# HENDRIX-ZT2/pyaudiorestoration

Measured on AMD Instinct MI355X. Metric: Msamples/sec resampled (192 kHz varispeed), higher is better.
Workload: dtype f32 near taps, far taps (|n| >= 3) as float16 hi + lo x 2^-12 filter banks on v_mfma_f32_16x16x32_f16 with f32 accumulation / f64 positions

## Files before the change

pyaudiorestoration_amd/csrc/sinc2.hip:

```cpp
#define PAR_WANT_BANK2 1
#include "par_common.h"
#include "pos_plan.h"
#include "sinc_taps_gen.h"
#include "sinc_common.h"
#define PAR_COLD_FN __forceinline__
#include "sinc_block.h"
#ifndef PAR_COLD_FN_GIVEN
#error "sinc_block.h was included before PAR_COLD_FN was defined: the cold functions would stay out of line"
#endif
#include <algorithm>
#include <atomic>
#include <limits.h>
#include <type_traits>

constexpr int kMaxTilesPerWave = 23;
#ifndef PAR_S2_EXP
#define PAR_S2_EXP 0
#endif

namespace par {

typedef _Float16 half8v __attribute__((ext_vector_type(8)));
typedef _Float16 half2v __attribute__((ext_vector_type(2)));
typedef float float4v __attribute__((ext_vector_type(4)));
// ... 138 lines not shown
  _Float16 img[2 * NCH][kRingH];
  float4v qa[kPass];
  float4v qm0[MOM ? kPass : kPass / 4];
  float4v qm1[MOM ? kPass : 1];
  __device__ __forceinline__ float& e2d2(int sl) {
    return MOM ? reinterpret_cast<float*>(&qm0[sl])[3] : reinterpret_cast<float*>(&qm0[0])[sl];
  }
  __device__ __forceinline__ const float& e2d2(int sl) const {
    return MOM ? reinterpret_cast<const float*>(&qm0[sl])[3] : reinterpret_cast<const float*>(&qm0[0])[sl];
  }
#ifdef PAR_S3_LDS_PAD
  uint4 pad[PAR_S3_LDS_PAD / 16];
#endif
  uint4 recs[4][16];
};
static_assert(offsetof(S3Lds<1>, img) % 16 == 0 && offsetof(S3Lds<1>, qa) % 16 == 0 && offsetof(S3Lds<1>, recs) % 16 == 0, "16-byte aligned");
static_assert(offsetof(S3Lds<2>, ring) % 16 == 0 && offsetof(S3Lds<2>, img) % 16 == 0 && offsetof(S3Lds<2>, qa) % 16 == 0 &&
              offsetof(S3Lds<2>, recs) % 16 == 0, "16-byte aligned");
static_assert(sizeof(S3Lds<2>) <= 20480, "eight stereo streams per compute unit (160 KB of LDS)");
using S3LdsUnity = S3Lds<1, false>;
static_assert(sizeof(S3LdsUnity) <= 10240 && offsetof(S3LdsUnity, recs) % 16 == 0 && offsetof(S3LdsUnity, qa) % 16 == 0,
              "sixteen fc = 1 streams per compute unit");

struct S3Pass {
  int cw[2];
  float s[2], ep[2];
  int nok[2];
  int j, ws;
};

constexpr int kCtabUnity = 10;
struct S3Frags {
  half8v xh[3], xl[3];
};
template <class LDS>
__device__ __forceinline__ S3Frags bank_load(const LDS& L, const int offs, const int l, const int ch = 0) {
  const int bb = l & 15, g = l >> 4;
  const int i0 = offs + 8 * bb + 8 * g;
  S3Frags X;
#pragma unroll
  for (int ks = 0; ks < 3; ++ks) {
    const int ix = (i0 + 32 * ks) & (kRingH - 1);
    X.xh[ks] = *reinterpret_cast<const half8v*>(&L.img[2 * ch][ix]);
    X.xl[ks] = *reinterpret_cast<const half8v*>(&L.img[2 * ch + 1][ix]);
  }
  return X;
}
template <bool MOMENTS, bool SIX = true, class LDS>
__device__ __forceinline__ void bank_math(LDS& L, const half8v (&fr)[kBank2Frags], const half8v (&fmr)[kBank3Frags],
                                          const S3Frags& X, const int l) {
  const int bb = l & 15, g = l >> 4;
  const half8v (&xh)[3] = X.xh, (&xl)[3] = X.xl;
  auto frag = [&](int f) { return f < kCtabUnity ? fr[f] : fmr[f - kCtabUnity]; };
  const float4v z = {0.0f, 0.0f, 0.0f, 0.0f};
  float4v e0 = z, lo = z, e1 = z, e2 = z;
#pragma unroll
  for (int ks = 0; ks < 3; ++ks) {
    const half8v f0 = frag(ks);
    e0 = __builtin_amdgcn_mfma_f32_16x16x32_f16(f0, xh[ks], e0, 0, 0, 0);
    lo = __builtin_amdgcn_mfma_f32_16x16x32_f16(frag(5 + ks), xh[ks], lo, 0, 0, 0);
    lo = __builtin_amdgcn_mfma_f32_16x16x32_f16(f0, xl[ks], lo, 0, 0, 0);
    if (ks < 2) {
      const half8v f1 = frag(3 + ks);
      e1 = __builtin_amdgcn_mfma_f32_16x16x32_f16(f1, xh[ks], e1, 0, 0, 0);
      e2 = __builtin_amdgcn_mfma_f32_16x16x32_f16(frag(8 + ks), xh[ks], e2, 0, 0, 0);
    }
  }
  float lo_inv = kBank2LoInv;
  asm volatile("" : "+v"(lo_inv));
  const float4v v0 = e0 + lo * lo_inv, v1 = e1;
  float4v a01 = z, l01 = z, a23 = z, a45 = z, a6 = z;
  if (MOMENTS) {
#pragma unroll
    for (int ks = 0; ks < 3; ++ks) {
      const half8v f01 = frag(kCtabUnity + ks);
      a01 = __builtin_amdgcn_mfma_f32_16x16x32_f16(f01, xh[ks], a01, 0, 0, 0);
      l01 = __builtin_amdgcn_mfma_f32_16x16x32_f16(frag(kCtabUnity + 3 + ks), xh[ks], l01, 0, 0, 0);
      l01 = __builtin_amdgcn_mfma_f32_16x16x32_f16(f01, xl[ks], l01, 0, 0, 0);
      a23 = __builtin_amdgcn_mfma_f32_16x16x32_f16(frag(kCtabUnity + 6 + ks), xh[ks], a23, 0, 0, 0);
      a45 = __builtin_amdgcn_mfma_f32_16x16x32_f16(frag(kCtabUnity + 9 + ks), xh[ks], a45, 0, 0, 0);
      if constexpr (SIX) a6 = __builtin_amdgcn_mfma_f32_16x16x32_f16(frag(kCtabUnity + 12 + ks), xh[ks], a6, 0, 0, 0);
    }
  }
  const float4v m01 = a01 + l01 * lo_inv;
#pragma unroll
  for (int p = 0; p < 2; ++p) {
    const int sl = (8 * bb + 2 * g + p) ^ (bb & 7);
    const float4v row = {v0[2 * p], v0[2 * p + 1], v1[2 * p], v1[2 * p + 1]};
    L.qa[sl] = row;
    const float e2d2 = __uint_as_float(pack_h2(e2[2 * p] * 0.015625f, e2[2 * p + 1] * 0.015625f));
    if constexpr (MOMENTS) {
      const float4v r0 = {m01[2 * p], m01[2 * p + 1], a23[2 * p], e2d2};
      L.qm0[sl] = r0;
      const float4v r1 = {a23[2 * p + 1], a45[2 * p], a45[2 * p + 1], a6[2 * p]};
      L.qm1[sl] = r1;
    } else {
      L.e2d2(sl) = e2d2;
    }
  }
}
template <bool MOMENTS, bool SIX = true, class LDS>
__device__ __forceinline__ void bank_image3m(LDS& L, const half8v (&fr)[kBank2Frags], const half8v (&fmr)[kBank3Frags],
                                             const int offs, const int l, const int ch = 0) {
  bank_math<MOMENTS, SIX>(L, fr, fmr, bank_load(L, offs, l, ch), l);
}

struct S3Gather {
  float4v row, M0, Mh;
  float xm2, xm1, x0, xp1, xp2;
};
template <int MODE, int NCH = 1, class LDS>
__device__ __forceinline__ S3Gather s3_out_load(const LDS& L, const int ci, const int wsK, const int ch = 0) {
  const int sl = ci ^ ((ci >> 3) & 7);
  const int rc = (wsK + ci) & (kRingF - 1);
  const float* xp = &L.ring[NCH * rc + ch];
  S3Gather G;
  G.xm2 = xp[-2 * NCH], G.xm1 = xp[-NCH], G.x0 = xp[0], G.xp1 = xp[NCH], G.xp2 = xp[2 * NCH];
  G.row = L.qa[sl];
  G.M0 = float4v{0.0f, 0.0f, 0.0f, 0.0f};
  G.Mh = G.M0;
  if constexpr (MODE != 1) {
    G.M0 = L.qm0[sl];
    G.Mh = L.qm1[sl];
  } else {
    G.M0[3] = L.e2d2(sl);
  }
  return G;
}
template <int MODE>
__device__ __forceinline__ float s3_out_math(const S3Gather& Gr, const float sr, const float epr) {
  using T32 = TapTab<32>;
  constexpr float kUs = kBank2ScaleInv * kImgScaleInv;
  constexpr float kMs = kImgScaleInv;
  const float xm2 = Gr.xm2, xm1 = Gr.xm1, x0 = Gr.x0, xp1 = Gr.xp1, xp2 = Gr.xp2;
  const float q = sr * sr, q64 = 64.0f * q;
  const float R1 = fast_rcp(fmaf(q, T32::B[1], T32::A[1])), R2 = fast_rcp(fmaf(q, T32::B[2], T32::A[2]));
  {
// ... 142 lines not shown
                                         jw, nrem, piece);
    else if (nrem > 0)
      fused_wave<NCH, 32, 2 * NCH, false>(a.len_out, a.sig, a.sig + 1, NCH, a.len_in, 32, a.tab, a.tmd, a.out, a.out + 1, NCH, a.fa, piece, l,
                                          jw, nrem, piece);
    return;
    }
  }
  const int64_t stream_id = (int64_t)bx - a.n_edge;
  const int my_tiles = stream_id < a.n_big ? a.tiles : a.tiles_tail;
  const int64_t Ta = stream_id < a.n_big ? stream_id * a.tiles : a.n_big * a.tiles + (stream_id - a.n_big) * a.tiles_tail;
  if (Ta >= a.n_full) return;
  const int64_t Tb = Ta + my_tiles < a.n_full ? Ta + my_tiles : a.n_full;
  const int64_t Ja = Ta * kSincTileOutputs, Jb = Tb * kSincTileOutputs;
  long long A0;
  int hd_dA, hd_fl;
  {
    const int64_t Ti = Ta + l < a.n_tiles ? Ta + l : a.n_tiles - 1;
    const TileHdr h = a.hdr[l <= my_tiles ? Ti : Ta];
    A0 = (long long)(((unsigned long long)(unsigned)__builtin_amdgcn_readfirstlane((int)((unsigned long long)h.anchor >> 32)) << 32) |
                     (unsigned)__builtin_amdgcn_readfirstlane((int)(unsigned)(unsigned long long)h.anchor));
    const long long d = h.anchor - A0;
    hd_fl = h.flags | ((d > -0x40000000ll && d < 0x40000000ll) ? 0 : 1);
    if (a.n_edge > 0 && (Ta + l == 0 || Ta + l >= a.n_full - 2)) hd_fl |= 1 | kTileEdge;
    hd_dA = (int)d;
    if constexpr (KIND == 1 || KIND == 2) {
      const bool any_slow = __ballot(l < my_tiles && Ta + l < Tb && (h.flags & kTileMaySlow) != 0) != 0ull;
      if (any_slow != (KIND == 2)) return;
    }
  }
  half8v fr[kBank2Frags];
  {
    const uint4* src = reinterpret_cast<const uint4*>(kBank2Frags32) + l;
#pragma unroll
    for (int f = 0; f < kBank2Frags; ++f) fr[f] = __builtin_bit_cast(half8v, src[f * kWave]);
  }
  half8v fmr[kBank3Frags];
  if constexpr (kMom) {
    const uint4* src = reinterpret_cast<const uint4*>(kBank3Frags32) + l;
#pragma unroll
    for (int f = 0; f < kBank3Frags; ++f) fmr[f] = __builtin_bit_cast(half8v, src[f * kWave]);
  }
  {
    uint4* z = reinterpret_cast<uint4*>(&L.img[0][0]);
    const uint4 zero = {0u, 0u, 0u, 0u};
#pragma unroll
    for (int i = 0; i < (int)(sizeof(L.img) / 16 / kWave); ++i) z[i * kWave + l] = zero;
  }
  const float tolf = (float)((fabs((double)A0) + 2.0e7) * 1.2e-16 + 2.0e-10) + 2.0e-7f;
  const int nJ = (int)(Jb - Ja);
  float* const outW = a.out + (kPick ? a.out_stride : (int64_t)NCH) * Ja;
  const uint4* const recW = reinterpret_cast<const uint4*>(a.rec) + (Ja >> kRecShift);
  const uint4* const rec2W = reinterpret_cast<const uint4*>(a.rec2) + (Ja >> kRecShift);
  const int blk_max = (int)(((a.len_out + kRec - 1) >> kRecShift) - (Ja >> kRecShift)) - 1;

  int j0 = 0;
  constexpr int kDmaBadMax = 1 << 22;
  int wbase = 0, conv_next = 0, conv_lo = 0, dma_next = 0, dma_bad = 0, mode = 0, pk = 0;
  int regime = 1;
  int rbA = 0, rbB = 0, rbC = 0;

  const uint4* const rec_lane = (l < 8 ? recW : rec2W) + (l & 7);
  using LdsT = S3Lds<NCH, KIND != 1>;
  const unsigned lds_base = lds_addr(&L);
  const unsigned lds_recs = lds_base + (unsigned)offsetof(LdsT, recs), lds_ring = lds_base + (unsigned)offsetof(LdsT, ring);
  constexpr unsigned kRecBufBytes = 16 * sizeof(uint4);
  constexpr unsigned kChunkBytes = kPass * NCH * sizeof(float);
  auto fetch_records_at = [&](unsigned rbytes, int blk0) {
    if (l < 16) dma_dwordx4(rec_lane + (blk0 < 0 ? 0 : blk0), lds_recs + rbytes);
  };
  auto fetch_records = [&](int buf, int blk0) { fetch_records_at(kRecBufBytes * (unsigned)buf, blk0); };
  unsigned long long ring_src = (unsigned long long)(uintptr_t)a.sig;
  auto ring_restart = [&]() {
    const long long o = A0 + wbase;
    ring_src = (unsigned long long)(uintptr_t)a.sig + (unsigned long long)((long long)(NCH * sizeof(float)) * o);
// ... 108 lines not shown
                "the largest stream (48 tiles of stereo frames) stays below 2^32 bytes");
  auto out_bytes = [&](auto elem, int j) -> size_t { return (size_t)(((unsigned)j + (unsigned)l) * (unsigned)sizeof(elem)); };
  auto store_pass = [&](const S3Pass& Q, const float (&res)[2]) {
#pragma unroll
    for (int r = 0; r < 2; ++r)
      if (l < Q.nok[r] && !(PAR_S2_EXP & 4)) {
        if constexpr (kPick) outW[(int64_t)((unsigned)Q.j + 64u * r + (unsigned)l) * a.out_stride] = res[r];
        else *reinterpret_cast<float*>(reinterpret_cast<char*>(outW) + out_bytes(float{}, Q.j) + kWave * sizeof(float) * r) = res[r];
      }
  };
  auto store_pass2 = [&](const S3Pass& Q, const float (&res0)[2], const float (&res1)[2]) {
#pragma unroll
    for (int r = 0; r < 2; ++r)
      if (l < Q.nok[r] && !(PAR_S2_EXP & 4))
        *reinterpret_cast<float2*>(reinterpret_cast<char*>(outW) + out_bytes(float2{}, Q.j) + kWave * sizeof(float2) * r) = make_float2(res0[r], res1[r]);
  };
  auto convert_chunk = [&](int w0) -> unsigned long long {
    if constexpr (kPick) {
      return s3_convert_ch(L, w0, l, 0, true);
    } else if constexpr (NCH == 2) {
      const unsigned long long t0 = s3_convert_ch(L, w0, l, 0, true);
      const unsigned long long t1 = s3_convert_ch(L, w0, l, 1, false);
      return t0 | t1;
    } else {
      return s3_convert(L, w0, l);
    }
  };

#if PAR_S2_EXP & 128
#define S3_COUNT(k) do { if (l == 0) atomicAdd(a.redo_count + (k), 1); } while (0)
#else
#define S3_COUNT(k) do { } while (0)
#endif
  auto start_run = [&]() -> bool {
    for (;;) {
      if (j0 >= nJ) return false;
      S3_COUNT(1);
      __builtin_amdgcn_s_waitcnt(0x0F70);
      wave_lds_fence();
      const int buf = pk & 3;
      fetch_records(buf, j0 >> kRecShift);
      __builtin_amdgcn_s_waitcnt(0x0F70);
      wave_lds_fence();
      const Placed Q = place(j0, buf, j0 >> kRecShift);
      const int tend = Q.tend;
      int nv[2] = {clamp64(nJ - j0), clamp64(nJ - j0 - 64)};
      const unsigned long long b0 = __ballot(Q.R[0].bad() || !(Q.R[0].ep <= kEpMaxMom)) & prefix(nv[0]),
                               b1 = __ballot(Q.R[1].bad() || !(Q.R[1].ep <= kEpMaxMom)) & prefix(nv[1]);
      const int nt0 = clamp64(Q.nt[0]), nt1 = clamp64(Q.nt[1]);
      const unsigned long long bad_here = (b0 & prefix(nt0)) | (b1 & prefix(nt1));
      const bool bad_next = ((b0 & ~prefix(nt0)) | (b1 & ~prefix(nt1)) | (unsigned long long)((Q.fl1 & 1) && tend < nJ)) != 0ull;
      if (bad_next) {
        nv[0] = nv[0] < nt0 ? nv[0] : nt0;
        nv[1] = nv[1] < nt1 ? nv[1] : nt1;
      }
      bool skip = (Q.fl0 & 1) || bad_here != 0ull;
      const unsigned long long gen = (__ballot(1.0f + Q.R[0].ep != 1.0f) & prefix(nv[0])) | (__ballot(1.0f + Q.R[1].ep != 1.0f) & prefix(nv[1]));
      const int ws = __builtin_amdgcn_readfirstlane(Q.R[0].c) & ~7;
      S3Pass N;
#pragma unroll
      for (int r = 0; r < 2; ++r) {
        N.cw[r] = Q.R[r].c - ws;
        N.s[r] = Q.R[r].s;
        N.ep[r] = Q.R[r].ep;
        const unsigned long long in = __ballot(N.cw[r] < kPass);
        N.nok[r] = __popcll(in & prefix(nv[r]));
      }
      N.j = j0;
      N.ws = ws;
// ... 27 lines not shown
        while (dma_next < conv_end + 2) chunk_dma(dma_next++);
        const int jn = j0 + N.nok[0] + N.nok[1];
        rbA = jn >> kRecShift;
        rbB = (jn + 120) >> kRecShift;
        fetch_records((pk + 1) & 3, rbA);
        fetch_records((pk + 2) & 3, rbB);
        __builtin_amdgcn_s_waitcnt(0x0F70);
        wave_lds_fence();
        if (!skip) {
#pragma unroll 1
          while (conv_next < conv_end) {
            if (conv_next >= dma_bad) {
              skip = true;
              break;
            }
            const bool ok = convert_chunk(kPass * conv_next) == 0ull;
            if (!ok) {
              skip = true;
              break;
            }
            ++conv_next;
          }
        }
        if (!skip && conv_next + 1 >= dma_bad) skip = true;
      }
      if (skip) {
        if (!(Q.fl0 & kTileEdge)) push_tile(Ta + (j0 >> 10));
        j0 = tend;
        mode = 0;
        continue;
      }
      wave_lds_fence();
      const int offs = ws - wbase - 31;
      if (kMom && regime == 3) bank_image3m<kMom, true>(L, fr, fmr, offs, l);
      else if (kMom && regime == 2) bank_image3m<kMom, false>(L, fr, fmr, offs, l);
      else bank_image3m<false>(L, fr, fmr, offs, l);
      wave_lds_fence();
      j0 += N.nok[0] + N.nok[1];
      ++pk;
      rbC = (j0 + 240) >> kRecShift;
      const bool full = N.nok[1] >= 1 && N.nok[0] + N.nok[1] >= 120;
      if (full) {
        P = N;
        return true;
      }
      float res[2];
      if (kMom && regime == 3) out_pass(std::integral_constant<int, kMom ? 3 : 1>{}, N, res);
      else if (kMom && regime == 2) out_pass(std::integral_constant<int, kMom ? 2 : 1>{}, N, res);
      else out_pass(std::integral_constant<int, 1>{}, N, res);
      if constexpr (kTwo) {
        float res1[2];
        wave_lds_fence();
        if (regime == 3) bank_image3m<true, true>(L, fr, fmr, offs, l, 1);
        else if (regime == 2) bank_image3m<true, false>(L, fr, fmr, offs, l, 1);
        else bank_image3m<false>(L, fr, fmr, offs, l, 1);
        wave_lds_fence();
        if (regime == 3) out_pass(std::integral_constant<int, 3>{}, N, res1, 1);
        else if (regime == 2) out_pass(std::integral_constant<int, 2>{}, N, res1, 1);
        else out_pass(std::integral_constant<int, 1>{}, N, res1, 1);
        store_pass2(N, res, res1);
      } else {
        store_pass(N, res);
      }
    }
  };

#if PAR_S2_EXP & 64
  unsigned long long s3t_[4] = {0, 0, 0, 0}, s3last_ = __builtin_readcyclecounter();
  const unsigned long long s3start_ = s3last_;
#endif
  auto hot = [&](auto mode_tag) {
    constexpr int MODE = decltype(mode_tag)::value;
    j0 = __builtin_amdgcn_readfirstlane(j0);
    wbase = __builtin_amdgcn_readfirstlane(wbase);
    rbA = __builtin_amdgcn_readfirstlane(rbA);
    rbB = __builtin_amdgcn_readfirstlane(rbB);
    rbC = __builtin_amdgcn_readfirstlane(rbC);
    tc_tend = __builtin_amdgcn_readfirstlane(tc_tend);
    tc_flm = __builtin_amdgcn_readfirstlane(tc_flm);
    const int cn0 = __builtin_amdgcn_readfirstlane(conv_next), pk0 = __builtin_amdgcn_readfirstlane(pk);
    const int dn0 = __builtin_amdgcn_readfirstlane(dma_next), dbad = __builtin_amdgcn_readfirstlane(dma_bad);
    int w0 = kPass * cn0;
    unsigned rbytes = kRecBufBytes * (unsigned)(pk0 & 3);
    unsigned dslot = kChunkBytes * (unsigned)(dn0 & 7);
    unsigned long long dsrc = ring_src + (unsigned long long)((long long)kChunkBytes * dn0);
    dsrc = ((unsigned long long)(unsigned)__builtin_amdgcn_readfirstlane((int)(dsrc >> 32)) << 32) |
           (unsigned)__builtin_amdgcn_readfirstlane((int)(unsigned)dsrc);
    const int nJm = nJ - kPass;
    const int cn_lim = kPass * (dbad - 2);
    const int dn_lim = kPass * (dbad - (dn0 - cn0));
    unsigned long long cok = 0ull;
    int m = 0, adv = 0;
    for (;;) {
#if PAR_S2_EXP & 64
      const unsigned long long tA_ = __builtin_readcyclecounter();
#endif
      if constexpr (NCH == 2) asm volatile("s_waitcnt vmcnt(7)" ::: "memory");
      else asm volatile("s_waitcnt vmcnt(5)" ::: "memory");
#if PAR_S2_EXP & 64
      const unsigned long long tB_ = __builtin_readcyclecounter();
      s3t_[0] += tB_ - tA_;
      s3t_[1] += tA_ - s3last_;
      s3last_ = tB_;
      s3t_[2] += 1;
#endif
// ... 18 lines not shown
        N.nok[r] = __popcll(__ballot(N.cw[r] < kPass));
      }
      N.j = j0;
      N.ws = ws;
      wsK = ws - wbase;
      const int d = w0 - wsK;
      auto smin = [](int x, int y) {
        int r = min(x, y);
        asm volatile("" : "+s"(r));
        return r;
      };
      adv = N.nok[0] + N.nok[1];
      m = smin(tc_flm, nJm - j0);
      m = smin(m, adv - 120 - 16 * n_none);
      m = smin(m, smin(d - 161, 473 - d));
      m = smin(m, cn_lim - w0);
      m = smin(m, smin(jb, 1 - jb));
      if constexpr (MODE != 1) m = smin(m, n_some - 1);
      };
      float res[2];
      if constexpr (kEarly) {
        const PlaceRecs RR = place_load(j0, rbytes, jb);
        const float2 cxx = s3_convert_load(L, w0, l);
        S3Gather G[2];
        const int wsP = P.ws - wbase;
#pragma unroll
        for (int r = 0; r < 2; ++r) {
          int ci = P.cw[r];
          ci = ci < 0 ? 0 : (ci > kPass - 1 ? kPass - 1 : ci);
          G[r] = s3_out_load<MODE, NCH>(L, ci, wsP);
        }
        __builtin_amdgcn_sched_barrier(0);
        place_next(std::true_type{}, RR);
        const S3Frags X = bank_load(L, wsK - 31, l);
        __builtin_amdgcn_sched_barrier(0);
        if constexpr (MODE == 2) {
          res[0] = s3_out_math<MODE>(G[0], P.s[0], P.ep[0]);
          asm volatile("" : "+v"(res[0]));
          asm volatile("" ::"v"(G[0].Mh[3]));
          __builtin_amdgcn_sched_barrier(0);
          res[1] = s3_out_math<MODE>(G[1], P.s[1], P.ep[1]);
          bank_math<true, false>(L, fr, fmr, X, l);
          asm volatile("" : "+v"(res[1]));
          asm volatile("" ::"v"(G[1].Mh[3]));
#pragma unroll
          for (int i = 0; i < 28; ++i) {
            __builtin_amdgcn_sched_group_barrier(0x008, 1, 0);
            __builtin_amdgcn_sched_group_barrier(0x002, 2, 0);
          }
        } else {
#pragma unroll
          for (int r = 0; r < 2; ++r) res[r] = s3_out_math<MODE>(G[r], P.s[r], P.ep[r]);
          asm volatile("" : "+v"(res[0]), "+v"(res[1]));
          __builtin_amdgcn_sched_barrier(0);
          bank_math<MODE != 1, MODE == 3>(L, fr, fmr, X, l);
        }
        cok = s3_convert_math(L, w0, l, cxx);
        fetch_records_at(rbytes ^ (2 * kRecBufBytes), rbC);
        chunk_dma_at(w0 < dn_lim, dsrc, dslot);
        store_pass(P, res);
      } else {
      if constexpr (!kTwo) place_next(std::false_type{}, PlaceRecs{});
      out_pass(mode_tag, P, res);
      if constexpr (kTwo) {
        float res1[2];
        asm volatile("" : "+v"(res[0]), "+v"(res[1]));
        bank_image3m<MODE != 1, MODE == 3>(L, fr, fmr, P.ws - wbase - 31, l, 1);
        out_pass(mode_tag, P, res1, 1);
        asm volatile("" : "+v"(res1[0]), "+v"(res1[1]));
        place_next(std::false_type{}, PlaceRecs{});
        const int offs = wsK - 31;
        bank_image3m<MODE != 1, MODE == 3>(L, fr, fmr, offs, l, 0);
        const unsigned long long c0 = s3_convert_ch(L, w0, l, 0, true);
        const unsigned long long c1 = s3_convert_ch(L, w0 - kPass, l, 1, false);
        cok = c0 | c1;
        fetch_records_at(rbytes ^ (2 * kRecBufBytes), rbC);
        chunk_dma_at(w0 < dn_lim, dsrc, dslot);
        store_pass2(P, res, res1);
      } else {
        const int offs = wsK - 31;
#if PAR_S3_PIN_MONO
        asm volatile("" : "+v"(res[0]), "+v"(res[1]));
#endif
        bank_image3m<MODE != 1, MODE == 3>(L, fr, fmr, offs, l);
        cok = convert_chunk(w0);
        fetch_records_at(rbytes ^ (2 * kRecBufBytes), rbC);
        chunk_dma_at(w0 < dn_lim, dsrc, dslot);
        store_pass(P, res);
      }
      }
      wave_lds_fence();
      w0 += kPass;
      dsrc += kChunkBytes;
      dslot = (dslot + kChunkBytes) & (8 * kChunkBytes - 1);
      S3_COUNT(2);
      if (min(m, -(int)__popcll(cok)) < 0) break;
      P = N;
      j0 += adv;
      rbytes = (rbytes + kRecBufBytes) & (3 * kRecBufBytes);
      rbA = rbB;
      rbB = rbC;
      rbC = (j0 + 240) >> kRecShift;
    }
    conv_next = w0 >> 7;
    dma_next = dn0 + (conv_next - cn0);
    pk = pk0 + (conv_next - cn0) - 1;
    if (cok != 0ull) mode = 0;
    if constexpr (kTwo)
      if (mode != 0 && s3_convert_ch(L, w0 - kPass, l, 1, false) != 0ull) mode = 0;
  };

  while (start_run()) {
    if (kMom && regime == 3) hot(std::integral_constant<int, kMom ? 3 : 1>{});
    else if (kMom && regime == 2) hot(std::integral_constant<int, kMom ? 2 : 1>{});
    else hot(std::integral_constant<int, 1>{});
  }
  __builtin_amdgcn_s_waitcnt(0x0F70);
#if PAR_S2_EXP & 64
  if (l == 0) {
    unsigned long long* o = g_s2_phase + (size_t)stream_id * 16;
    o[0] = s3t_[0];
    o[1] = s3t_[1];
    o[2] = s3t_[2];
    o[3] = __builtin_readcyclecounter() - s3start_;
    o[6] = s3t_[2];
  }
#endif
}

template <int NCH, int KIND>
__global__ __launch_bounds__(kWave, KIND == 1 ? 3 : 2) void k_sinc_pipe(const S2Args a) {
  __shared__ S3Lds<NCH, KIND != 1> L;
  sinc_pipe_body<NCH, KIND>(a, (int)blockIdx.x, L);
}

constexpr int kBatchFiles = kFusedBatchMax;
struct S2Batch {
  int n;
  int first[kBatchFiles + 1];
  S2Args f[kBatchFiles];
};
static_assert(sizeof(S2Batch) <= 3584, "kernel arguments fit the 4 KB segment");
template <int NCH, int KIND>
__global__ __launch_bounds__(kWave, KIND == 1 ? 3 : 2) void k_sinc_pipe_n(const S2Batch b) {
  __shared__ S3Lds<NCH, KIND != 1> L;
  const int bx = (int)blockIdx.x;
  int fi = 0;
// ... 107 lines not shown
```

pyaudiorestoration_amd/csrc/sinc_taps_gen.h:

```cpp
#pragma once

namespace par {

template <int NT> struct TapTab;

template <> struct TapTab<32> {
  static constexpr int p1_from = 9, p0_from = 25;
  static constexpr int mode[33] = {0, 0, 0, 0, 0, 1, 1, 1, 1, 2, 2, 2, 2, 2, 2, 2, 2, 2, 2, 2, 2, 2, 2, 2, 2, 3, 3, 3, 3, 3, 3, 3, 3};
  static constexpr float A[33] = {0.0f, 3.149174690246582f, 12.688271522521973f, 28.89647102355957f, 52.254295349121094f, -0.011980682611465454f, 0.008096873760223389f, -0.005758844781666994f, 0.0042452262714505196f, -0.0032113760244101286f, 0.0024757650680840015f, -0.001935371314175427f, 0.0015282001113519073f, -0.0012151190312579274f, 0.0009704310796223581f, -0.000776688102632761f, 0.0006216989131644368f, -0.0004967301501892507f, 0.0003953868872486055f, -0.0003128938842564821f, 0.0002456224465277046f, -0.00019077055912930518f, 0.00014614294923376292f, -0.00010999643563991413f, 8.092952339211479e-05f, -5.7813980674836785e-05f, 3.9685513911535963e-05f, -2.5783318051253445e-05f, 1.5455205357284285e-05f, -8.15003295429051e-06f, 3.398380613361951e-06f, -7.97579900790879e-07f, 0.0f};
  static constexpr float B[33] = {-3.1415927410125732f, -3.149174690246582f, -3.172067880630493f, -3.210718870162964f, -3.2658934593200684f, -0.00047922731027938426f, 0.00022491315030492842f, -0.00011752743739634752f, 6.633166049141437e-05f, -3.976941297878511e-05f, 2.481971932866145e-05f, -1.6027928722905926e-05f, 1.0630960787239019e-05f, -7.2007073868007865e-06f, 4.957503279001685e-06f, -3.4557874641905073e-06f, 2.4308856154675595e-06f, -1.7202777371494449e-06f, 1.221272327711631e-06f, -8.673427487337904e-07f, 6.144401254459808e-07f, -4.328316833834833e-07f, 3.0210429713406484e-07f, -2.0803109634925931e-07f, 1.40563656714221e-07f, 0.0f, 0.0f, 0.0f, 0.0f, 0.0f, 0.0f, 0.0f, 0.0f};
  static constexpr float C[33] = {0.0f, 0.0f, 0.0f, 0.0f, 0.0f, -1.916909241117537e-05f, 6.247587862162618e-06f, -2.398519200141891e-06f, 1.0364321951783495e-06f, 0.0f, 0.0f, 0.0f, 0.0f, 0.0f, 0.0f, 0.0f, 0.0f, 0.0f, 0.0f, 0.0f, 0.0f, 0.0f, 0.0f, 0.0f, 0.0f, 0.0f, 0.0f, 0.0f, 0.0f, 0.0f, 0.0f, 0.0f, 0.0f};
};

template <> struct TapTab<50> {
  static constexpr int p1_from = 9, p0_from = 37;
  static constexpr int mode[51] = {0, 0, 0, 0, 0, 1, 1, 1, 1, 2, 2, 2, 2, 2, 2, 2, 2, 2, 2, 2, 2, 2, 2, 2, 2, 2, 2, 2, 2, 2, 2, 2, 2, 2, 2, 2, 2, 3, 3, 3, 3, 3, 3, 3, 3, 3, 3, 3, 3, 3, 3};
  static constexpr float A[51] = {0.0f, 3.144695281982422f, 12.616111755371094f, 28.526979446411133f, 51.06767654418945f, -0.01242081169039011f, 0.008531484752893448f, -0.006186992395669222f, 0.004665991757065058f, -0.0036238711327314377f, 0.0028791376389563084f, -0.0023288081865757704f, 0.0019109291024506092f, -0.0015864137094467878f, 0.0013296125689521432f, -0.0011231281096115708f, 0.000954821880441159f, -0.0008160152356140316f, 0.0007003697683103383f, -0.0006031683878973126f, 0.0005208412767387927f, -0.00045064662117511034f, 0.0003904495679307729f, -0.0003385677409823984f, 0.00029366035596467555f, -0.0002546478935983032f, 0.00022065313532948494f, -0.0001909568381961435f, 0.0001649646437726915f, -0.0001421815832145512f, 0.00012219262134749442f, -0.00010464734805282205f, 8.924811118049547e-05f, -7.574055780423805e-05f, 6.39061036054045e-05f, -5.355593020794913e-05f, 4.452605207916349e-05f, -3.667675264296122e-05f, 2.987515108543448e-05f, -2.4015091184992343e-05f, 1.8998915038537234e-05f, -1.473993052059086e-05f, 1.1160883332195226e-05f, -8.192681889340747e-06f, 5.773316843260545e-06f, -3.846952040476026e-06f, 2.3631571366422577e-06f, -1.2762477581418352e-06f, 5.447275839287613e-07f, -1.3080894234462903e-07f, 0.0f};
  static constexpr float B[51] = {-3.1415927410125732f, -3.144695281982422f, -3.1540279388427734f, -3.1696643829345703f, -3.191729784011841f, -0.0004968324792571366f, 0.0002369856956647709f, -0.00012626514944713563f, 7.290612120414153e-05f, -4.4877713662572205e-05f, 2.8863558327429928e-05f, -1.9286206224933267e-05f, 1.3293425581650808e-05f, -9.400972885487135e-06f, 6.792402928113006e-06f, -4.9972336455539335e-06f, 3.7334193621063605e-06f, -2.826027184710256e-06f, 2.163304543500999e-06f, -1.6719844779800042e-06f, 1.3029175534029491e-06f, -1.0224540574199636e-06f, 8.071309025581286e-07f, -6.403172392310807e-07f, 5.10048380419903e-07f, -4.075996855590347e-07f, 3.265307384481275e-07f, -2.6203341008113057e-07f, 2.10481204021562e-07f, -1.6911280908971094e-07f, 1.358072978518976e-07f, -1.0892255630778891e-07f, 8.717763932963862e-08f, -6.956653209044816e-08f, 5.5294055556487365e-08f, -4.37280505138915e-08f, 3.4363150547278565e-08f, 0.0f, 0.0f, 0.0f, 0.0f, 0.0f, 0.0f, 0.0f, 0.0f, 0.0f, 0.0f, 0.0f, 0.0f, 0.0f, 0.0f};
  static constexpr float C[51] = {0.0f, 0.0f, 0.0f, 0.0f, 0.0f, -1.9873297787853517e-05f, 6.58293583910563e-06f, -2.5768399609660264e-06f, 1.1391581438147114e-06f, 0.0f, 0.0f, 0.0f, 0.0f, 0.0f, 0.0f, 0.0f, 0.0f, 0.0f, 0.0f, 0.0f, 0.0f, 0.0f, 0.0f, 0.0f, 0.0f, 0.0f, 0.0f, 0.0f, 0.0f, 0.0f, 0.0f, 0.0f, 0.0f, 0.0f, 0.0f, 0.0f, 0.0f, 0.0f, 0.0f, 0.0f, 0.0f, 0.0f, 0.0f, 0.0f, 0.0f, 0.0f, 0.0f, 0.0f, 0.0f, 0.0f, 0.0f};
};

constexpr int kFarrowFrags = 10;
constexpr float kFarrowScaleInv = 0.03125f, kFarrowLoInv = 0.000244140625f;
#ifdef __HIPCC__
// ... 1081 lines not shown
  0x9df71c4au, 0xa1312000u, 0xa3f62287u, 0xa56824b6u, 0x00000000u, 0x00000000u, 0x00000000u, 0x00000000u, 0x1c4a99f0u, 0x20009df7u, 0x2287a131u, 0x24b6a3f6u,
  0x00000000u, 0x00000000u, 0x00000000u, 0x00000000u, 0x99f017e0u, 0x9df71c4au, 0xa1312000u, 0xa3f62287u, 0x00000000u, 0x00000000u, 0x00000000u, 0x00000000u,
  0x17e094f9u, 0x1c4a99f0u, 0x20009df7u, 0x2287a131u, 0x00000000u, 0x00000000u, 0x00000000u, 0x00000000u, 0x94f911efu, 0x99f017e0u, 0x9df71c4au, 0xa1312000u,
  0x00000000u, 0x00000000u, 0x00000000u, 0x00000000u, 0x2635a69bu, 0x245fa574u, 0x1eaea21bu, 0x00009813u, 0x00000000u, 0x00000000u, 0x00000000u, 0x00000000u,
  0xa69b26acu, 0xa5742635u, 0xa21b245fu, 0x98131eaeu, 0x00000000u, 0x00000000u, 0x00000000u, 0x00000000u, 0x26aca674u, 0x2635a69bu, 0x245fa574u, 0x1eaea21bu,
  0x00000000u, 0x00000000u, 0x00000000u, 0x00000000u, 0xa6742602u, 0xa69b26acu, 0xa5742635u, 0xa21b245fu, 0x00000000u, 0x00000000u, 0x00000000u, 0x00000000u,
  0x2602a568u, 0x26aca674u, 0x2635a69bu, 0x245fa574u, 0x00000000u, 0x00000000u, 0x00000000u, 0x00000000u, 0xa56824b6u, 0xa6742602u, 0xa69b26acu, 0xa5742635u,
  0x00000000u, 0x00000000u, 0x00000000u, 0x00000000u, 0x24b6a3f6u, 0x2602a568u, 0x26aca674u, 0x2635a69bu, 0x00000000u, 0x00000000u, 0x00000000u, 0x00000000u,
  0xa3f62287u, 0xa56824b6u, 0xa6742602u, 0xa69b26acu, 0x00000000u, 0x00000000u, 0x00000000u, 0x00000000u, 0x00000000u, 0x00000000u, 0x00000000u, 0x00000000u,
  0x00000000u, 0x00000000u, 0x00000000u, 0x00000000u, 0x00000000u, 0x00000000u, 0x00000000u, 0x00000000u, 0x00000000u, 0x00000000u, 0x00000000u, 0x00000000u,
  0x00009813u, 0x00000000u, 0x00000000u, 0x00000000u, 0x00000000u, 0x00000000u, 0x00000000u, 0x00000000u, 0x98131eaeu, 0x00000000u, 0x00000000u, 0x00000000u,
  0x00000000u, 0x00000000u, 0x00000000u, 0x00000000u, 0x1eaea21bu, 0x00009813u, 0x00000000u, 0x00000000u, 0x00000000u, 0x00000000u, 0x00000000u, 0x00000000u,
  0xa21b245fu, 0x98131eaeu, 0x00000000u, 0x00000000u, 0x00000000u, 0x00000000u, 0x00000000u, 0x00000000u, 0x245fa574u, 0x1eaea21bu, 0x00009813u, 0x00000000u,
  0x00000000u, 0x00000000u, 0x00000000u, 0x00000000u, 0xa5742635u, 0xa21b245fu, 0x98131eaeu, 0x00000000u, 0x00000000u, 0x00000000u, 0x00000000u, 0x00000000u,
  0x00000000u, 0x00000000u, 0x00000000u, 0x00000000u, 0x00000000u, 0x00000000u, 0x00000000u, 0x00000000u, 0x00000000u, 0x00000000u, 0x00000000u, 0x00000000u,
  0x00000000u, 0x00000000u, 0x00000000u, 0x00000000u, 0x00000000u, 0x00000000u, 0x00000000u, 0x00000000u, 0x00000000u, 0x00000000u, 0x00000000u, 0x00000000u,
  0x00000000u, 0x00000000u, 0x00000000u, 0x00000000u, 0x00000000u, 0x00000000u, 0x00000000u, 0x00000000u, 0x00000000u, 0x00000000u, 0x00000000u, 0x00000000u,
  0x00000000u, 0x00000000u, 0x00000000u, 0x00000000u, 0x00000000u, 0x00000000u, 0x00000000u, 0x00000000u, 0x00000000u, 0x00000000u, 0x00000000u, 0x00000000u,
  0x00000000u, 0x00000000u, 0x00000000u, 0x00000000u, 0x00000000u, 0x00000000u, 0x00000000u, 0x00000000u, 0x00000000u, 0x00000000u, 0x00000000u, 0x00000000u,
  0x00000000u, 0x00000000u, 0x00000000u, 0x00000000u, 0x00000000u, 0x00000000u, 0x00000000u, 0x00000000u, 0x00000000u, 0x00000000u, 0x00000000u, 0x00000000u,
  0x00000000u, 0x00000000u, 0x00000000u, 0x00000000u, 0x00000000u, 0x00000000u, 0x00000000u, 0x00000000u, 0x00000000u, 0x00000000u, 0x00000000u, 0x00000000u,
  0x00000000u, 0x00000000u, 0x00000000u, 0x00000000u, 0x00000000u, 0x00000000u, 0x00000000u, 0x00000000u, 0x00000000u, 0x00000000u, 0x00000000u, 0x00000000u,
  0x00000000u, 0x00000000u, 0x00000000u, 0x00000000u, 0x00000000u, 0x00000000u, 0x00000000u, 0x00000000u, 0x00000000u, 0x00000000u, 0x00000000u, 0x00000000u,
  0x00000000u, 0x00000000u, 0x00000000u, 0x00000000u, 0x00000000u, 0x00000000u, 0x00000000u, 0x00000000u, 0x00000000u, 0x00000000u, 0x00000000u, 0x00000000u,
  0x00000000u, 0x00000000u, 0x00000000u, 0x00000000u, 0x00000000u, 0x00000000u, 0x00000000u, 0x00000000u, 0x00000000u, 0x00000000u, 0x00000000u, 0x00000000u,
  0x00000000u, 0x00000000u, 0x00000000u, 0x00000000u, 0x00000000u, 0x00000000u, 0x00000000u, 0x00000000u, 0x00000000u, 0x00000000u, 0x00000000u, 0x00000000u,
  0x00000000u, 0x00000000u, 0x00000000u, 0x00000000u, 0x00000000u, 0x00000000u, 0x00000000u, 0x00000000u, 0x00000000u, 0x00000000u, 0x00000000u, 0x00000000u,
  0x00000000u, 0x00000000u, 0x00000000u, 0x00000000u, 0x00000000u, 0x00000000u, 0x00000000u, 0x00000000u, 0x00000000u, 0x00000000u, 0x00000000u, 0x00000000u,
  0x00000000u, 0x00000000u, 0x00000000u, 0x00000000u, 0x00000000u, 0x00000000u, 0x00000000u, 0x00000000u, 0x00000000u, 0x00000000u, 0x00000000u, 0x00000000u,
  0x00000000u, 0x00000000u, 0x00000000u, 0x00000000u, 0x00000000u, 0x00000000u, 0x00000000u, 0x00000000u, 0x00000000u, 0x00000000u, 0x00000000u, 0x00000000u,
};
#endif

}
```

Baseline: 187,700.

## Fold third k-step lo-correction MFMAs into one combined fragment for non-six modes

In the filter-bank MFMA routine, the third k-slice's hi/lo correction products (lo and l01 accumulators) are replaced by one MFMA that uses a precomputed fold fragment and a single extra LDS load spanning the hi and lo images. This happens in modes other than the full six-moment one. It removes several MFMAs and LDS loads per bank image in modes 1 and 2. The cost is extra register fragments (fsw), reloading the swap fragments when switching into or out of regime 3, and a retuned sched_group_barrier count. The restructured start_run/finish control flow and the new regime return codes add complexity and risk of mode-dependent mistakes.

Result: faster. 191,700, median of 6 (+2.1%).

```diff
diff --git a/pyaudiorestoration_amd/csrc/sinc2.hip b/pyaudiorestoration_amd/csrc/sinc2.hip
--- a/pyaudiorestoration_amd/csrc/sinc2.hip
+++ b/pyaudiorestoration_amd/csrc/sinc2.hip
@@ -194,30 +194,52 @@
 constexpr int kCtabUnity = 10;
 struct S3Frags {
   half8v xh[3], xl[3];
+  half8v xv;
 };
-template <class LDS>
-__device__ __forceinline__ S3Frags bank_load(const LDS& L, const int offs, const int l, const int ch = 0) {
+struct S3XvLane {
+  unsigned at, img;
+};
+__device__ __forceinline__ S3XvLane bank_xv_img(const int l) {
+  return S3XvLane{16u * (unsigned)(l & 15) + 64u * (unsigned)sizeof(_Float16), (l >> 4) == 2 ? (unsigned)(kRingH * sizeof(_Float16)) : 0u};
+}
+template <bool FOLD, bool XH2, class LDS>
+__device__ __forceinline__ S3Frags bank_load(const LDS& L, const int offs, const int l, const S3XvLane xv_img, const int ch = 0) {
   const int bb = l & 15, g = l >> 4;
-  const int i0 = offs + 8 * bb + 8 * g;
+  constexpr unsigned kImgBytes = kRingH * sizeof(_Float16);
+  const unsigned b0 = (unsigned)offs * (unsigned)sizeof(_Float16) + 16u * (unsigned)(bb + g);
+  const char* const hi = reinterpret_cast<const char*>(&L.img[2 * ch][0]);
+  const char* const lo = reinterpret_cast<const char*>(&L.img[2 * ch + 1][0]);
   S3Frags X;
 #pragma unroll
   for (int ks = 0; ks < 3; ++ks) {
-    const int ix = (i0 + 32 * ks) & (kRingH - 1);
-    X.xh[ks] = *reinterpret_cast<const half8v*>(&L.img[2 * ch][ix]);
-    X.xl[ks] = *reinterpret_cast<const half8v*>(&L.img[2 * ch + 1][ix]);
+    const unsigned at = (b0 + 64u * ks) & (kImgBytes - 1u);
+    X.xh[ks] = X.xl[ks] = half8v{};
+    if (ks < 2 || !FOLD || XH2) X.xh[ks] = *reinterpret_cast<const half8v*>(hi + at);
+    if (ks < 2 || !FOLD) X.xl[ks] = *reinterpret_cast<const half8v*>(lo + at);
+  }
+  X.xv = half8v{};
+  if constexpr (FOLD) {
+    static_assert(sizeof(L.img[0]) == kImgBytes, "the lo image lies kImgBytes behind the hi image");
+    const unsigned at = (((unsigned)offs * (unsigned)sizeof(_Float16) + xv_img.at) & (kImgBytes - 1u)) | xv_img.img;
+    X.xv = *reinterpret_cast<const half8v*>(hi + at);
   }
   return X;
 }
+constexpr bool bank_folds(bool moments, bool six) { return !(moments && six); }
 template <bool MOMENTS, bool SIX = true, class LDS>
 __device__ __forceinline__ void bank_math(LDS& L, const half8v (&fr)[kBank2Frags], const half8v (&fmr)[kBank3Frags],
-                                          const S3Frags& X, const int l) {
+                                          const half8v (&fsw)[4], const S3Frags& X, const int l) {
+  constexpr bool FOLD = bank_folds(MOMENTS, SIX);
+  constexpr int NS = FOLD ? 2 : 3;
   const int bb = l & 15, g = l >> 4;
   const half8v (&xh)[3] = X.xh, (&xl)[3] = X.xl;
-  auto frag = [&](int f) { return f < kCtabUnity ? fr[f] : fmr[f - kCtabUnity]; };
+  auto frag = [&](int f) {
+    return f == 2 ? fsw[0] : f == 7 ? fsw[1] : f == kCtabUnity + 2 ? fsw[2] : f == kCtabUnity + 5 ? fsw[3] : f < kCtabUnity ? fr[f] : fmr[f - kCtabUnity];
+  };
   const float4v z = {0.0f, 0.0f, 0.0f, 0.0f};
   float4v e0 = z, lo = z, e1 = z, e2 = z;
 #pragma unroll
-  for (int ks = 0; ks < 3; ++ks) {
+  for (int ks = 0; ks < NS; ++ks) {
     const half8v f0 = frag(ks);
     e0 = __builtin_amdgcn_mfma_f32_16x16x32_f16(f0, xh[ks], e0, 0, 0, 0);
     lo = __builtin_amdgcn_mfma_f32_16x16x32_f16(frag(5 + ks), xh[ks], lo, 0, 0, 0);
@@ -228,17 +250,21 @@
       e2 = __builtin_amdgcn_mfma_f32_16x16x32_f16(frag(8 + ks), xh[ks], e2, 0, 0, 0);
     }
   }
+  if constexpr (FOLD) lo = __builtin_amdgcn_mfma_f32_16x16x32_f16(fsw[0], X.xv, lo, 0, 0, 0);
   float lo_inv = kBank2LoInv;
   asm volatile("" : "+v"(lo_inv));
   const float4v v0 = e0 + lo * lo_inv, v1 = e1;
   float4v a01 = z, l01 = z, a23 = z, a45 = z, a6 = z;
   if (MOMENTS) {
+    if constexpr (FOLD) l01 = __builtin_amdgcn_mfma_f32_16x16x32_f16(fsw[1], X.xv, l01, 0, 0, 0);
 #pragma unroll
     for (int ks = 0; ks < 3; ++ks) {
-      const half8v f01 = frag(kCtabUnity + ks);
-      a01 = __builtin_amdgcn_mfma_f32_16x16x32_f16(f01, xh[ks], a01, 0, 0, 0);
-      l01 = __builtin_amdgcn_mfma_f32_16x16x32_f16(frag(kCtabUnity + 3 + ks), xh[ks], l01, 0, 0, 0);
-      l01 = __builtin_amdgcn_mfma_f32_16x16x32_f16(f01, xl[ks], l01, 0, 0, 0);
+      if (ks < NS) {
+        const half8v f01 = frag(kCtabUnity + ks);
+        a01 = __builtin_amdgcn_mfma_f32_16x16x32_f16(f01, xh[ks], a01, 0, 0, 0);
+        l01 = __builtin_amdgcn_mfma_f32_16x16x32_f16(frag(kCtabUnity + 3 + ks), xh[ks], l01, 0, 0, 0);
+        l01 = __builtin_amdgcn_mfma_f32_16x16x32_f16(f01, xl[ks], l01, 0, 0, 0);
+      }
       a23 = __builtin_amdgcn_mfma_f32_16x16x32_f16(frag(kCtabUnity + 6 + ks), xh[ks], a23, 0, 0, 0);
       a45 = __builtin_amdgcn_mfma_f32_16x16x32_f16(frag(kCtabUnity + 9 + ks), xh[ks], a45, 0, 0, 0);
       if constexpr (SIX) a6 = __builtin_amdgcn_mfma_f32_16x16x32_f16(frag(kCtabUnity + 12 + ks), xh[ks], a6, 0, 0, 0);
@@ -263,8 +289,8 @@
 }
 template <bool MOMENTS, bool SIX = true, class LDS>
 __device__ __forceinline__ void bank_image3m(LDS& L, const half8v (&fr)[kBank2Frags], const half8v (&fmr)[kBank3Frags],
-                                             const int offs, const int l, const int ch = 0) {
-  bank_math<MOMENTS, SIX>(L, fr, fmr, bank_load(L, offs, l, ch), l);
+                                             const half8v (&fsw)[4], const int offs, const int l, const S3XvLane xv_img, const int ch = 0) {
+  bank_math<MOMENTS, SIX>(L, fr, fmr, fsw, bank_load<bank_folds(MOMENTS, SIX), MOMENTS>(L, offs, l, xv_img, ch), l);
 }
 
 struct S3Gather {
@@ -473,14 +499,31 @@
   {
     const uint4* src = reinterpret_cast<const uint4*>(kBank2Frags32) + l;
 #pragma unroll
-    for (int f = 0; f < kBank2Frags; ++f) fr[f] = __builtin_bit_cast(half8v, src[f * kWave]);
+    for (int f = 0; f < kBank2Frags; ++f) fr[f] = f == 2 || f == 7 ? half8v{} : __builtin_bit_cast(half8v, src[f * kWave]);
   }
   half8v fmr[kBank3Frags];
   if constexpr (kMom) {
     const uint4* src = reinterpret_cast<const uint4*>(kBank3Frags32) + l;
 #pragma unroll
-    for (int f = 0; f < kBank3Frags; ++f) fmr[f] = __builtin_bit_cast(half8v, src[f * kWave]);
-  }
+    for (int f = 0; f < kBank3Frags; ++f) fmr[f] = f == 2 || f == 5 ? half8v{} : __builtin_bit_cast(half8v, src[f * kWave]);
+  }
+  half8v fsw[4] = {half8v{}, half8v{}, half8v{}, half8v{}};
+  auto fsw_load = [&](bool six) {
+    int ll = l;
+    asm volatile("" : "+v"(ll));
+    const uint4* const b2 = reinterpret_cast<const uint4*>(kBank2Frags32) + ll;
+    const uint4* const b3 = reinterpret_cast<const uint4*>(kBank3Frags32) + ll;
+    if (six) {
+      fsw[0] = __builtin_bit_cast(half8v, b2[2 * kWave]);
+      fsw[1] = __builtin_bit_cast(half8v, b2[7 * kWave]);
+      fsw[2] = __builtin_bit_cast(half8v, b3[2 * kWave]);
+      fsw[3] = __builtin_bit_cast(half8v, b3[5 * kWave]);
+    } else {
+      fsw[0] = __builtin_bit_cast(half8v, reinterpret_cast<const uint4*>(kBank2FoldFrag32)[ll]);
+      if constexpr (kMom) fsw[1] = __builtin_bit_cast(half8v, reinterpret_cast<const uint4*>(kBank3FoldFrag32)[ll]);
+    }
+  };
+  fsw_load(false);
   {
     uint4* z = reinterpret_cast<uint4*>(&L.img[0][0]);
     const uint4 zero = {0u, 0u, 0u, 0u};
@@ -655,9 +698,9 @@
 #else
 #define S3_COUNT(k) do { } while (0)
 #endif
-  auto start_run = [&]() -> bool {
+  auto start_run = [&]() -> int {
     for (;;) {
-      if (j0 >= nJ) return false;
+      if (j0 >= nJ) return 0;
       S3_COUNT(1);
       __builtin_amdgcn_s_waitcnt(0x0F70);
       wave_lds_fence();
@@ -751,35 +794,48 @@
       }
       wave_lds_fence();
       const int offs = ws - wbase - 31;
-      if (kMom && regime == 3) bank_image3m<kMom, true>(L, fr, fmr, offs, l);
-      else if (kMom && regime == 2) bank_image3m<kMom, false>(L, fr, fmr, offs, l);
-      else bank_image3m<false>(L, fr, fmr, offs, l);
-      wave_lds_fence();
-      j0 += N.nok[0] + N.nok[1];
-      ++pk;
-      rbC = (j0 + 240) >> kRecShift;
       const bool full = N.nok[1] >= 1 && N.nok[0] + N.nok[1] >= 120;
-      if (full) {
-        P = N;
-        return true;
-      }
-      float res[2];
-      if (kMom && regime == 3) out_pass(std::integral_constant<int, kMom ? 3 : 1>{}, N, res);
-      else if (kMom && regime == 2) out_pass(std::integral_constant<int, kMom ? 2 : 1>{}, N, res);
-      else out_pass(std::integral_constant<int, 1>{}, N, res);
-      if constexpr (kTwo) {
-        float res1[2];
+      auto finish = [&](auto mode_tag) {
+        constexpr int MODE = decltype(mode_tag)::value;
+        bank_image3m<MODE != 1, MODE == 3>(L, fr, fmr, fsw, offs, l, bank_xv_img(l));
         wave_lds_fence();
-        if (regime == 3) bank_image3m<true, true>(L, fr, fmr, offs, l, 1);
-        else if (regime == 2) bank_image3m<true, false>(L, fr, fmr, offs, l, 1);
-        else bank_image3m<false>(L, fr, fmr, offs, l, 1);
-        wave_lds_fence();
-        if (regime == 3) out_pass(std::integral_constant<int, 3>{}, N, res1, 1);
-        else if (regime == 2) out_pass(std::integral_constant<int, 2>{}, N, res1, 1);
-        else out_pass(std::integral_constant<int, 1>{}, N, res1, 1);
-        store_pass2(N, res, res1);
+        j0 += N.nok[0] + N.nok[1];
+        ++pk;
+        rbC = (j0 + 240) >> kRecShift;
+        if (full) return;
+        float res[2];
+        out_pass(mode_tag, N, res);
+        if constexpr (kTwo) {
+          float res1[2];
+          wave_lds_fence();
+          bank_image3m<MODE != 1, MODE == 3>(L, fr, fmr, fsw, offs, l, bank_xv_img(l), 1);
+          wave_lds_fence();
+          out_pass(mode_tag, N, res1, 1);
+          store_pass2(N, res, res1);
+        } else {
+          store_pass(N, res);
+        }
+      };
+      if (kMom && regime == 3) {
+        fsw_load(true);
+        finish(std::integral_constant<int, kMom ? 3 : 1>{});
+        if (full) {
+          P = N;
+          return 3;
+        }
+        fsw_load(false);
+      } else if (kMom && regime == 2) {
+        finish(std::integral_constant<int, kMom ? 2 : 1>{});
+        if (full) {
+          P = N;
+          return 2;
+        }
       } else {
-        store_pass(N, res);
+        finish(std::integral_constant<int, 1>{});
+        if (full) {
+          P = N;
+          return 1;
+        }
       }
     }
   };
@@ -790,6 +846,11 @@
 #endif
   auto hot = [&](auto mode_tag) {
     constexpr int MODE = decltype(mode_tag)::value;
+    S3XvLane xv_img = {0u, 0u};
+    if constexpr (MODE != 3) {
+      xv_img = bank_xv_img(l);
+      asm volatile("" : "+v"(xv_img.at), "+v"(xv_img.img));
+    }
     j0 = __builtin_amdgcn_readfirstlane(j0);
     wbase = __builtin_amdgcn_readfirstlane(wbase);
     rbA = __builtin_amdgcn_readfirstlane(rbA);
@@ -874,7 +935,7 @@
         }
         __builtin_amdgcn_sched_barrier(0);
         place_next(std::true_type{}, RR);
-        const S3Frags X = bank_load(L, wsK - 31, l);
+        const S3Frags X = bank_load<MODE != 3, MODE != 1>(L, wsK - 31, l, xv_img);
         __builtin_amdgcn_sched_barrier(0);
         if constexpr (MODE == 2) {
           res[0] = s3_out_math<MODE>(G[0], P.s[0], P.ep[0]);
@@ -882,20 +943,26 @@
           asm volatile("" ::"v"(G[0].Mh[3]));
           __builtin_amdgcn_sched_barrier(0);
           res[1] = s3_out_math<MODE>(G[1], P.s[1], P.ep[1]);
-          bank_math<true, false>(L, fr, fmr, X, l);
+          bank_math<true, false>(L, fr, fmr, fsw, X, l);
           asm volatile("" : "+v"(res[1]));
           asm volatile("" ::"v"(G[1].Mh[3]));
 #pragma unroll
-          for (int i = 0; i < 28; ++i) {
+          for (int i = 0; i < 24; ++i) {
             __builtin_amdgcn_sched_group_barrier(0x008, 1, 0);
             __builtin_amdgcn_sched_group_barrier(0x002, 2, 0);
           }
         } else {
 #pragma unroll
-          for (int r = 0; r < 2; ++r) res[r] = s3_out_math<MODE>(G[r], P.s[r], P.ep[r]);
+          for (int r = 0; r < 2; ++r) {
+            res[r] = s3_out_math<MODE>(G[r], P.s[r], P.ep[r]);
+            if constexpr (MODE == 3) {
+              asm volatile("" : "+v"(res[r]));
+              __builtin_amdgcn_sched_barrier(0);
+            }
+          }
           asm volatile("" : "+v"(res[0]), "+v"(res[1]));
           __builtin_amdgcn_sched_barrier(0);
-          bank_math<MODE != 1, MODE == 3>(L, fr, fmr, X, l);
+          bank_math<MODE != 1, MODE == 3>(L, fr, fmr, fsw, X, l);
         }
         cok = s3_convert_math(L, w0, l, cxx);
         fetch_records_at(rbytes ^ (2 * kRecBufBytes), rbC);
@@ -907,12 +974,12 @@
       if constexpr (kTwo) {
         float res1[2];
         asm volatile("" : "+v"(res[0]), "+v"(res[1]));
-        bank_image3m<MODE != 1, MODE == 3>(L, fr, fmr, P.ws - wbase - 31, l, 1);
+        bank_image3m<MODE != 1, MODE == 3>(L, fr, fmr, fsw, P.ws - wbase - 31, l, xv_img, 1);
         out_pass(mode_tag, P, res1, 1);
         asm volatile("" : "+v"(res1[0]), "+v"(res1[1]));
         place_next(std::false_type{}, PlaceRecs{});
         const int offs = wsK - 31;
-        bank_image3m<MODE != 1, MODE == 3>(L, fr, fmr, offs, l, 0);
+        bank_image3m<MODE != 1, MODE == 3>(L, fr, fmr, fsw, offs, l, xv_img, 0);
         const unsigned long long c0 = s3_convert_ch(L, w0, l, 0, true);
         const unsigned long long c1 = s3_convert_ch(L, w0 - kPass, l, 1, false);
         cok = c0 | c1;
@@ -924,7 +991,7 @@
 #if PAR_S3_PIN_MONO
         asm volatile("" : "+v"(res[0]), "+v"(res[1]));
 #endif
-        bank_image3m<MODE != 1, MODE == 3>(L, fr, fmr, offs, l);
+        bank_image3m<MODE != 1, MODE == 3>(L, fr, fmr, fsw, offs, l, xv_img);
         cok = convert_chunk(w0);
         fetch_records_at(rbytes ^ (2 * kRecBufBytes), rbC);
         chunk_dma_at(w0 < dn_lim, dsrc, dslot);
@@ -952,9 +1019,11 @@
       if (mode != 0 && s3_convert_ch(L, w0 - kPass, l, 1, false) != 0ull) mode = 0;
   };
 
-  while (start_run()) {
-    if (kMom && regime == 3) hot(std::integral_constant<int, kMom ? 3 : 1>{});
-    else if (kMom && regime == 2) hot(std::integral_constant<int, kMom ? 2 : 1>{});
+  while (const int run = start_run()) {
+    if (kMom && run == 3) {
+      hot(std::integral_constant<int, kMom ? 3 : 1>{});
+      fsw_load(false);
+    } else if (kMom && run == 2) hot(std::integral_constant<int, kMom ? 2 : 1>{});
     else hot(std::integral_constant<int, 1>{});
   }
   __builtin_amdgcn_s_waitcnt(0x0F70);
diff --git a/pyaudiorestoration_amd/csrc/sinc_taps_gen.h b/pyaudiorestoration_amd/csrc/sinc_taps_gen.h
--- a/pyaudiorestoration_amd/csrc/sinc_taps_gen.h
+++ b/pyaudiorestoration_amd/csrc/sinc_taps_gen.h
@@ -1137,4 +1137,55 @@
 };
 #endif
 
+#ifdef PAR_WANT_BANK2
+__device__ const unsigned int kBank2FoldFrag32[256] = {
+  0x00000000u, 0x00000000u, 0x00000000u, 0x00000000u, 0x00000000u, 0x00000000u, 0x00000000u, 0x00000000u, 0x00000000u, 0x00000000u, 0x00000000u, 0x00000000u,
+  0x00000000u, 0x00000000u, 0x00000000u, 0x00000000u, 0x0000c2b1u, 0x00000000u, 0x00000000u, 0x00000000u, 0x0000d67bu, 0x00000000u, 0x00000000u, 0x00000000u,
+  0xc2b14b20u, 0x00000000u, 0x00000000u, 0x00000000u, 0xd67b5eaeu, 0x00000000u, 0x00000000u, 0x00000000u, 0x4b20d046u, 0x0000c2b1u, 0x00000000u, 0x00000000u,
+  0x5eaee3bfu, 0x0000d67bu, 0x00000000u, 0x00000000u, 0xd046540du, 0xc2b14b20u, 0x00000000u, 0x00000000u, 0xe3bf6717u, 0xd67b5eaeu, 0x00000000u, 0x00000000u,
+  0x540dd6c2u, 0x4b20d046u, 0x0000c2b1u, 0x00000000u, 0x6717e9b4u, 0x5eaee3bfu, 0x0000d67bu, 0x00000000u, 0xd6c25934u, 0xd046540du, 0xc2b14b20u, 0x00000000u,
+  0xe9b46c3au, 0xe3bf6717u, 0xd67b5eaeu, 0x00000000u, 0x00000000u, 0x00000000u, 0x00000000u, 0x00000000u, 0x00000000u, 0x00000000u, 0x00000000u, 0x00000000u,
+  0x00000000u, 0x00000000u, 0x00000000u, 0x00000000u, 0x00000000u, 0x00000000u, 0x00000000u, 0x00000000u, 0x00000ebau, 0x00000000u, 0x00000000u, 0x00000000u,
+  0x0000a43eu, 0x00000000u, 0x00000000u, 0x00000000u, 0x0eba1bdeu, 0x00000000u, 0x00000000u, 0x00000000u, 0xa43e2f60u, 0x00000000u, 0x00000000u, 0x00000000u,
+  0x1bde1bc0u, 0x00000ebau, 0x00000000u, 0x00000000u, 0x2f603183u, 0x0000a43eu, 0x00000000u, 0x00000000u, 0x1bc021cdu, 0x0eba1bdeu, 0x00000000u, 0x00000000u,
+  0x31832c4du, 0xa43e2f60u, 0x00000000u, 0x00000000u, 0x21cda4a0u, 0x1bde1bc0u, 0x00000ebau, 0x00000000u, 0x2c4d3063u, 0x2f603183u, 0x0000a43eu, 0x00000000u,
+  0xa4a0aa01u, 0x1bc021cdu, 0x0eba1bdeu, 0x00000000u, 0x3063b305u, 0x31832c4du, 0xa43e2f60u, 0x00000000u, 0x00000000u, 0x00000000u, 0x00000000u, 0x00000000u,
+  0x00000000u, 0x00000000u, 0x00000000u, 0x00000000u, 0x00000000u, 0x00000000u, 0x00000000u, 0x00000000u, 0x00000000u, 0x00000000u, 0x00000000u, 0x00000000u,
+  0x000092b1u, 0x00000000u, 0x00000000u, 0x00000000u, 0x0000a67bu, 0x00000000u, 0x00000000u, 0x00000000u, 0x92b11b20u, 0x00000000u, 0x00000000u, 0x00000000u,
+  0xa67b2eaeu, 0x00000000u, 0x00000000u, 0x00000000u, 0x1b20a046u, 0x000092b1u, 0x00000000u, 0x00000000u, 0x2eaeb3bfu, 0x0000a67bu, 0x00000000u, 0x00000000u,
+  0xa046240du, 0x92b11b20u, 0x00000000u, 0x00000000u, 0xb3bf3717u, 0xa67b2eaeu, 0x00000000u, 0x00000000u, 0x240da6c2u, 0x1b20a046u, 0x000092b1u, 0x00000000u,
+  0x3717b9b4u, 0x2eaeb3bfu, 0x0000a67bu, 0x00000000u, 0xa6c22934u, 0xa046240du, 0x92b11b20u, 0x00000000u, 0xb9b43c3au, 0xb3bf3717u, 0xa67b2eaeu, 0x00000000u,
+  0x00000000u, 0x00000000u, 0x00000000u, 0x00000000u, 0x00000000u, 0x00000000u, 0x00000000u, 0x00000000u, 0x00000000u, 0x00000000u, 0x00000000u, 0x00000000u,
+  0x00000000u, 0x00000000u, 0x00000000u, 0x00000000u, 0x00000000u, 0x00000000u, 0x00000000u, 0x00000000u, 0x00000000u, 0x00000000u, 0x00000000u, 0x00000000u,
+  0x00000000u, 0x00000000u, 0x00000000u, 0x00000000u, 0x00000000u, 0x00000000u, 0x00000000u, 0x00000000u, 0x00000000u, 0x00000000u, 0x00000000u, 0x00000000u,
+  0x00000000u, 0x00000000u, 0x00000000u, 0x00000000u, 0x00000000u, 0x00000000u, 0x00000000u, 0x00000000u, 0x00000000u, 0x00000000u, 0x00000000u, 0x00000000u,
+  0x00000000u, 0x00000000u, 0x00000000u, 0x00000000u, 0x00000000u, 0x00000000u, 0x00000000u, 0x00000000u, 0x00000000u, 0x00000000u, 0x00000000u, 0x00000000u,
+  0x00000000u, 0x00000000u, 0x00000000u, 0x00000000u,
+};
+__device__ const unsigned int kBank3FoldFrag32[256] = {
+  0x00000000u, 0x00000000u, 0x00000000u, 0x00000000u, 0x00000000u, 0x00000000u, 0x00000000u, 0x00000000u, 0x00000000u, 0x00000000u, 0x00000000u, 0x00000000u,
+  0x00000000u, 0x00000000u, 0x00000000u, 0x00000000u, 0x0000c8eeu, 0x00000000u, 0x00000000u, 0x00000000u, 0x0000c8c7u, 0x00000000u, 0x00000000u, 0x00000000u,
+  0xc8ee50ebu, 0x00000000u, 0x00000000u, 0x00000000u, 0xc8c7509du, 0x00000000u, 0x00000000u, 0x00000000u, 0x50ebd583u, 0x0000c8eeu, 0x00000000u, 0x00000000u,
+  0x509dd4ffu, 0x0000c8c7u, 0x00000000u, 0x00000000u, 0xd58358dfu, 0xc8ee50ebu, 0x00000000u, 0x00000000u, 0xd4ff5843u, 0xc8c7509du, 0x00000000u, 0x00000000u,
+  0x58dfdb8fu, 0x50ebd583u, 0x0000c8eeu, 0x00000000u, 0x5843da60u, 0x509dd4ffu, 0x0000c8c7u, 0x00000000u, 0xdb8f5d65u, 0xd58358dfu, 0xc8ee50ebu, 0x00000000u,
+  0xda605c62u, 0xd4ff5843u, 0xc8c7509du, 0x00000000u, 0x00000000u, 0x00000000u, 0x00000000u, 0x00000000u, 0x00000000u, 0x00000000u, 0x00000000u, 0x00000000u,
+  0x00000000u, 0x00000000u, 0x00000000u, 0x00000000u, 0x00000000u, 0x00000000u, 0x00000000u, 0x00000000u, 0x000098b8u, 0x00000000u, 0x00000000u, 0x00000000u,
+  0x000014dbu, 0x00000000u, 0x00000000u, 0x00000000u, 0x98b82018u, 0x00000000u, 0x00000000u, 0x00000000u, 0x14dba32au, 0x00000000u, 0x00000000u, 0x00000000u,
+  0x20181558u, 0x000098b8u, 0x00000000u, 0x00000000u, 0xa32a24cdu, 0x000014dbu, 0x00000000u, 0x00000000u, 0x1558250cu, 0x98b82018u, 0x00000000u, 0x00000000u,
+  0x24cd2835u, 0x14dba32au, 0x00000000u, 0x00000000u, 0x250c2a5eu, 0x20181558u, 0x000098b8u, 0x00000000u, 0x2835a921u, 0xa32a24cdu, 0x000014dbu, 0x00000000u,
+  0x2a5eae62u, 0x1558250cu, 0x98b82018u, 0x00000000u, 0xa921ac30u, 0x24cd2835u, 0x14dba32au, 0x00000000u, 0x00000000u, 0x00000000u, 0x00000000u, 0x00000000u,
+  0x00000000u, 0x00000000u, 0x00000000u, 0x00000000u, 0x00000000u, 0x00000000u, 0x00000000u, 0x00000000u, 0x00000000u, 0x00000000u, 0x00000000u, 0x00000000u,
+  0x000098eeu, 0x00000000u, 0x00000000u, 0x00000000u, 0x000098c7u, 0x00000000u, 0x00000000u, 0x00000000u, 0x98ee20ebu, 0x00000000u, 0x00000000u, 0x00000000u,
+  0x98c7209du, 0x00000000u, 0x00000000u, 0x00000000u, 0x20eba583u, 0x000098eeu, 0x00000000u, 0x00000000u, 0x209da4ffu, 0x000098c7u, 0x00000000u, 0x00000000u,
+  0xa58328dfu, 0x98ee20ebu, 0x00000000u, 0x00000000u, 0xa4ff2843u, 0x98c7209du, 0x00000000u, 0x00000000u, 0x28dfab8fu, 0x20eba583u, 0x000098eeu, 0x00000000u,
+  0x2843aa60u, 0x209da4ffu, 0x000098c7u, 0x00000000u, 0xab8f2d65u, 0xa58328dfu, 0x98ee20ebu, 0x00000000u, 0xaa602c62u, 0xa4ff2843u, 0x98c7209du, 0x00000000u,
+  0x00000000u, 0x00000000u, 0x00000000u, 0x00000000u, 0x00000000u, 0x00000000u, 0x00000000u, 0x00000000u, 0x00000000u, 0x00000000u, 0x00000000u, 0x00000000u,
+  0x00000000u, 0x00000000u, 0x00000000u, 0x00000000u, 0x00000000u, 0x00000000u, 0x00000000u, 0x00000000u, 0x00000000u, 0x00000000u, 0x00000000u, 0x00000000u,
+  0x00000000u, 0x00000000u, 0x00000000u, 0x00000000u, 0x00000000u, 0x00000000u, 0x00000000u, 0x00000000u, 0x00000000u, 0x00000000u, 0x00000000u, 0x00000000u,
+  0x00000000u, 0x00000000u, 0x00000000u, 0x00000000u, 0x00000000u, 0x00000000u, 0x00000000u, 0x00000000u, 0x00000000u, 0x00000000u, 0x00000000u, 0x00000000u,
+  0x00000000u, 0x00000000u, 0x00000000u, 0x00000000u, 0x00000000u, 0x00000000u, 0x00000000u, 0x00000000u, 0x00000000u, 0x00000000u, 0x00000000u, 0x00000000u,
+  0x00000000u, 0x00000000u, 0x00000000u, 0x00000000u,
+};
+#endif
+
 }
```
